# Fro116/RecommenderSystem

Measured on AMD Instinct MI355X. Metric: interactions/sec, higher is better.
Workload: dtype bf16

## Files before the change

recommendersystem_amd/csrc/elementwise.hip:

```cpp
#include "kernels.hpp"

namespace rsys {

thread_local DetScratch g_det;

__global__ void reduce_parts_kernel(const float* __restrict__ part, int nparts, long long stride, int n, float* dst) {
  const int c = blockIdx.x * blockDim.x + threadIdx.x;
  if (c >= n) return;
  float acc = 0.f;
  for (int b = 0; b < nparts; ++b) acc += part[(long long)b * stride + c];
  dst[c] += acc;
}
__global__ void reduce_parts_stage_kernel(const float* __restrict__ part, int nparts, long long stride, int n, float* out) {
  const int c = blockIdx.x * blockDim.x + threadIdx.x, chunk = blockIdx.y;
  if (c >= n) return;
  const int b0 = chunk * 32, b1 = min(nparts, b0 + 32);
  float acc = 0.f;
  for (int b = b0; b < b1; ++b) acc += part[(long long)b * stride + c];
  out[(long long)chunk * n + c] = acc;
}
int launch_reduce_parts(const float* part, int nparts, long long stride, int n, float* dst, hipStream_t s) {
  if (nparts <= 0 || n <= 0) return RSYS_OK;
  if (nparts > 64 && g_det.tmp != nullptr) {
    const int chunks = (nparts + 31) / 32;
// ... 716 lines not shown
int launch_rowdot(const T* h, const float* w, const float* b, float* out, int n, int D, hipStream_t s) {
  hipLaunchKernelGGL((rowdot_kernel<T>), dim3(div_up(n, 4)), dim3(256), 0, s, h, w, b, out, n, D);
  HIP_CHECK(hipGetLastError());
  return RSYS_OK;
}
template int launch_rowdot<bf16>(const bf16*, const float*, const float*, float*, int, int, hipStream_t);
template int launch_rowdot<float>(const float*, const float*, const float*, float*, int, int, hipStream_t);

template <typename TS>
__global__ void colsum_kernel(const TS* __restrict__ src, long long ld, long long rows, int cols, float* dst, int rows_per_block, float* part) {
  const int c = blockIdx.x * blockDim.x + threadIdx.x;
  if (c >= cols) return;
  const long long r0 = (long long)blockIdx.y * rows_per_block, r1 = min(rows, r0 + rows_per_block);
  float acc = 0.f;
  for (long long r = r0; r < r1; ++r) acc += to_f32(src[r * ld + c]);
  if (part != nullptr) part[(long long)blockIdx.y * cols + c] = acc;
  else if (acc != 0.f) atomicAdd(&dst[c], acc);
}
template <typename TS>
static int colsum_any(const TS* src, long long ld, long long rows, int cols, float* dst, hipStream_t s) {
  int rpb = (int)std::max<long long>(64, (rows + 511) / 512);
  dim3 grid(div_up(cols, 256), div_up(rows, rpb));
  float* part = det_part((long long)grid.y * cols);
  hipLaunchKernelGGL((colsum_kernel<TS>), grid, dim3(256), 0, s, src, ld, rows, cols, dst, rpb, part);
  HIP_CHECK(hipGetLastError());
  if (part != nullptr) return launch_reduce_parts(part, (int)grid.y, cols, cols, dst, s);
  return RSYS_OK;
}
int launch_colsum_add(const float* src, long long ld, long long rows, int cols, float* dst, hipStream_t s) {
  return colsum_any<float>(src, ld, rows, cols, dst, s);
}

__global__ __launch_bounds__(1024) void cast_colsum_kernel(const float* __restrict__ src, bf16* __restrict__ dst, long long rows, int D,
                                                           float* colsum, int rows_per_block, float* part) {
  __shared__ float red[2048];
  const int cg = D >> 2;
  const int c = (threadIdx.x % cg) * 4, lane_r = threadIdx.x / cg, nr = 1024 / cg;
  const long long r0 = (long long)blockIdx.x * rows_per_block, r1 = min(rows, r0 + rows_per_block);
  float4 acc = make_float4(0, 0, 0, 0);
  long long r = r0 + lane_r;
  for (; r + 3 * nr < r1; r += 4 * nr) {
    float4 v[4];
#pragma unroll
    for (int u = 0; u < 4; ++u) v[u] = *(const float4*)(src + (r + u * nr) * D + c);
#pragma unroll
    for (int u = 0; u < 4; ++u) {
      bf16x4 o; o[0] = (bf16)v[u].x; o[1] = (bf16)v[u].y; o[2] = (bf16)v[u].z; o[3] = (bf16)v[u].w;
      *(bf16x4*)(dst + (r + u * nr) * D + c) = o;
      acc.x += v[u].x; acc.y += v[u].y; acc.z += v[u].z; acc.w += v[u].w;
    }
  }
  for (; r < r1; r += nr) {
    const float4 v = *(const float4*)(src + r * D + c);
    bf16x4 o; o[0] = (bf16)v.x; o[1] = (bf16)v.y; o[2] = (bf16)v.z; o[3] = (bf16)v.w;
    *(bf16x4*)(dst + r * D + c) = o;
    acc.x += v.x; acc.y += v.y; acc.z += v.z; acc.w += v.w;
  }
  if (lane_r < 2) *(float4*)&red[lane_r * D + c] = acc;
  __syncthreads();
  for (int base = 2; base < nr; base += 2) {
    if (lane_r >= base && lane_r < base + 2) {
      float4 o = *(float4*)&red[(lane_r - base) * D + c];
      o.x += acc.x; o.y += acc.y; o.z += acc.z; o.w += acc.w;
      *(float4*)&red[(lane_r - base) * D + c] = o;
    }
    __syncthreads();
  }
  for (int cc = threadIdx.x; cc < D; cc += 1024) {
    const float v = red[cc] + (nr > 1 ? red[D + cc] : 0.f);
    if (part != nullptr) part[(long long)blockIdx.x * D + cc] = v;
    else if (v != 0.f) atomicAdd(&colsum[cc], v);
  }
}
int launch_cast_colsum(const float* src, bf16* dst, long long rows, int D, float* colsum, hipStream_t s) {
  ARG_CHECK(D % 4 == 0 && D <= 1024 && 1024 % (D >> 2) == 0, "cast_colsum: D/4 must divide 1024, D <= 1024");
  const int rpb = (int)std::max<long long>(32, (rows + 511) / 512);
  const int grid = div_up(rows, rpb);
  float* part = det_part((long long)grid * D);
  hipLaunchKernelGGL(cast_colsum_kernel, dim3(grid), dim3(1024), 0, s, src, dst, rows, D, colsum, rpb, part);
  HIP_CHECK(hipGetLastError());
  if (part != nullptr) return launch_reduce_parts(part, grid, D, D, colsum, s);
  return RSYS_OK;
}

__global__ __launch_bounds__(256) void cast_transpose_colsum_kernel(const float* __restrict__ src, bf16* __restrict__ dstT, long long rows, int D,
                                                                    long long ldt, float* colsum, int rows_per_block, float* part) {
  __shared__ unsigned short tile[64][72];
  __shared__ float red[16][64];
  const int t = threadIdx.x;
  const int lr = t >> 4, c4 = (t & 15) * 4;
  const int oc = t >> 2, or8 = (t & 3) * 16;
  const long long r0 = (long long)blockIdx.x * rows_per_block;
  const long long rend = min((rows + 63) & ~63LL, r0 + rows_per_block);
  for (int ct = 0; ct < D / 64; ++ct) {
    float4 acc = make_float4(0, 0, 0, 0);
    for (long long rb = r0; rb < rend; rb += 64) {
      float4 v[4];
#pragma unroll
      for (int i = 0; i < 4; ++i) {
        const long long r = rb + 4 * lr + i;
        v[i] = r < rows ? *(const float4*)(src + r * D + ct * 64 + c4) : make_float4(0, 0, 0, 0);
        acc.x += v[i].x; acc.y += v[i].y; acc.z += v[i].z; acc.w += v[i].w;
      }
      {
        bf16x4 o;
        o[0] = (bf16)v[0].x; o[1] = (bf16)v[1].x; o[2] = (bf16)v[2].x; o[3] = (bf16)v[3].x; *(bf16x4*)&tile[c4 + 0][4 * lr] = o;
        o[0] = (bf16)v[0].y; o[1] = (bf16)v[1].y; o[2] = (bf16)v[2].y; o[3] = (bf16)v[3].y; *(bf16x4*)&tile[c4 + 1][4 * lr] = o;
        o[0] = (bf16)v[0].z; o[1] = (bf16)v[1].z; o[2] = (bf16)v[2].z; o[3] = (bf16)v[3].z; *(bf16x4*)&tile[c4 + 2][4 * lr] = o;
        o[0] = (bf16)v[0].w; o[1] = (bf16)v[1].w; o[2] = (bf16)v[2].w; o[3] = (bf16)v[3].w; *(bf16x4*)&tile[c4 + 3][4 * lr] = o;
      }
      __syncthreads();
      {
        const uint4 q0 = *(const uint4*)&tile[oc][or8], q1 = *(const uint4*)&tile[oc][or8 + 8];
        uint4* d = (uint4*)(dstT + (long long)(ct * 64 + oc) * ldt + rb + or8);
// ... 127 lines not shown
```

recommendersystem_amd/csrc/kernels.hpp:

```cpp
#pragma once
#include "common.hpp"

namespace rsys {

struct BatchDev {
  int N, rows, S;
  const int *userid, *tmid, *gender, *source, *matchedid, *status;
  const double* time;
  const float *rating, *progress;
  const float* label[6]; const float* weight[6]; const int* position[6];
  const unsigned char *watch_mask, *rating_mask;
  const int* rope_pos;
  int *m_tmid, *m_matchedid, *m_status;
  float *m_rating, *m_progress;
  float* m_label[4]; float* m_weight[4]; int* m_position[4];
};

struct DetScratch {
  float* part = nullptr; long long cap = 0; float* tmp = nullptr; long long tmp_cap = 0;
  int part_used = 0, part_short = 0;
};
extern thread_local DetScratch g_det;
int launch_reduce_parts(const float* part, int nparts, long long stride, int n, float* dst, hipStream_t s);

// ... 26 lines not shown
                       float* f8_amax = nullptr );
template <typename T>
int launch_rmsnorm_bwd_f32(const float* g, const float* x, const float* scale, const float* rstd, const float* resid_grad,
                           float* dx_out, T* dx_out_t, float* dscale, long long rows, int D, hipStream_t s, const int* rows_dev = nullptr,
                           float* f8_amax = nullptr);

template <typename T>
int launch_dropout(const T* src, T* dst, long long n, float p, unsigned long long seed, unsigned int stream, int accumulate, hipStream_t s);

int launch_select_positions(const float* w, int N, int topk, int* idx, float* stats ,
                            int* npos_out , hipStream_t s);
int launch_select_positions_chunked(int ntask, const float* const* w, int N, int topk, int* const* idx, float* const* stats, int* const* npos_out,
                                    void* scratch, hipStream_t s);
int launch_select_positions_batch(int ntask, const float* const* w, int N, int topk, int* const* idx, float* const* stats,
                                  int* const* npos_out, hipStream_t s);

template <typename T>
int launch_gather_rows(const T* src, long long ld, const int* idx, int parity, T* dst, int n, int D, hipStream_t s);

int launch_scatter_rows_add(const float* src, const int* idx, int parity, float* dst, long long ld, int n, int D, hipStream_t s,
                            const int* npos = nullptr );

template <typename T>
int launch_ce_fwd_bwd(T* logits, long long ldl, int n, int V, const int* idx, const float* label, const float* weight,
                      const int* position, const float* stats, const int* npos, float task_w, float* loss_out, hipStream_t s);

template <typename T>
int launch_rating_tail(T* z, const T* hact, int n, int D, const float* w2, const float* b2, const int* idx,
                       const float* label, const float* weight, const float* stats, float rating_mean, float task_w,
                       int evaluate, float* loss_out , float* dw2, float* db2, float* db0, hipStream_t s,
                       const int* npos = nullptr );

int launch_colsum_add(const float* src, long long ld, long long rows, int cols, float* dst, hipStream_t s);
int launch_cast_colsum(const float* src, bf16* dst, long long rows, int D, float* colsum, hipStream_t s);
int launch_cast_transpose_colsum(const float* src, bf16* dstT, long long rows, int D, long long ldt, float* colsum, hipStream_t s);

int launch_embedding_scatter_add(const float* gx0, const BatchDev& b, int V, int D, float* gE, hipStream_t s);

int token_index_capacity(int N);
int launch_token_index_build(const int* matchedid, int N, int V, unsigned long long* keys, int* skey, int* sidx, hipStream_t s);
size_t seg_scatter_slab_floats(int N, int D);
int launch_embedding_scatter_segmented(const float* gx0, long long ldx, const int* m_matchedid, const int* skey, const int* sidx,
                                       int N, int V, int D, float* gE, float* slab, hipStream_t s);

int launch_token_union(const int* const* idx, const int* const* npos, int ntask, int NT, unsigned int* bits, int* pre, int* nsel, hipStream_t s);
int launch_selected_first(const unsigned int* bits, const int* pre, int* slot, int* sel, const int* uid, const int* tm, const int* rope_pos, int B, int T,
                          int* perm, int* uid_p, int* tm_p, int* pos_p, int* slot_p, int* sel_p, int* q_active, hipStream_t s);
template <typename T> int launch_gather_rows_sel(const T* src, long long ld, const int* sel, const int* n_dev, int cap, T* dst, int D, hipStream_t s);
template <typename T> int launch_scatter_rows_fill(const T* src, const int* slot_p, const int* q_active, int B, int Tseq, T* dst, long long ld, int D, hipStream_t s);
template <typename T> int launch_scatter_rows_sel(const T* src, const int* sel, const int* n_dev, int cap, T* dst, long long ld, int D, hipStream_t s);
template <typename T> int launch_scatter_rows_map(const T* src, const int* map, int n, T* dst, long long ld, int D, hipStream_t s);
template <typename T> int launch_gather_rows_slot(const T* compact, const int* slot, const int* idx, int parity, T* dst, int n, int D, hipStream_t s);
int launch_scatter_rows_add_slot(const float* src, const int* slot, const int* idx, int parity, const int* npos, float* compact, int n, int D, hipStream_t s);

int launch_plan_unique(const int* skey, const int* sidx, int N, int V, int* slot, int* uniq, int* tok2u, int* plan , hipStream_t s);
int launch_plan_offsets(const int* uniq, const int* plan, const int* bound_dev, int nb, int* off, hipStream_t s);
int launch_gather_rows_by_id(const float* src, long long ld, const int* ids, int sub, float* dst, int n, int D, hipStream_t s);
int launch_add_rows_by_id(const float* src, const int* ids, int sub, float* dst, long long ld, int n, int D, hipStream_t s);
int launch_add_rows_by_id_counted(const float* src, const int* ids, const int* count_dev, float* dst, long long ld, int cap, int D, hipStream_t s);
int launch_gather_items_remote(const BatchDev& b, const float* Frem, const int* tok2u, const int* plan, int D, float* x0,
                               int* uid_t, int* tm_t, hipStream_t s);
int launch_vp_meta(const int* idx, const float* label, const float* weight, const int* position, const float* stats,
                   const int* npos, float task_w, int KB, int KBmax, float* own , hipStream_t s);
int launch_add_scalar(float* dst, const float* src, hipStream_t s);
template <typename T>
int launch_vp_compact(const T* EwAll, const float* metaAll, int W, int KB, int D, T* EwC, float* metaC, int* nlive, int* pre , hipStream_t s);
// ... 104 lines not shown
```

recommendersystem_amd/csrc/model.hip:

```cpp
#include "model_internal.hpp"

namespace rsys {

static void add_tensor(Model* m, const std::string& name, int64_t rows, int64_t cols, int ndim, int64_t off, int64_t ld,
                       int map, bool trainable = true, bool frozen = false) {
  TensorInfo t{name, rows, cols, ndim, off, ld, map, trainable, frozen};
  m->by_name[name] = (int)m->tensors.size();
  m->tensors.push_back(t);
}

static void build_layout(Model* m) {
  const int D = m->D, Ip = m->Ip, I = m->I, L = m->L, hd = m->hd, H = m->H, KV = m->KV;
  const bool ft = m->cfg.finetune != 0;
  int64_t off = 0;
  auto take = [&](int64_t n) { int64_t o = off; off += pad8(n); return o; };
  m->lo.resize(L);
  if (ft) {
    for (int l = 0; l < L; ++l) { m->lo[l].la = take((int64_t)16 * D); m->lo[l].lb = take((int64_t)m->Nqkv * 16); }
  }
  const int64_t n_lora = off;
  m->o_status = take((m->cfg.vocab_status + 1) * 16);
  m->o_gender = take((m->cfg.vocab_gender + 1) * 4);
  m->o_source = take((m->cfg.vocab_source + 1) * 4);
  m->o_lin_w = take((int64_t)D * 32);
// ... 30 lines not shown
  add_tensor(m, "item_embedding.projection_layer.bias", 1, D, 1, m->o_bp, D, MAP_DIRECT, tr);
  for (int l = 0; l < L; ++l) {
    std::string p = "transformers.layers." + std::to_string(l) + ".";
    add_tensor(m, p + "attn.q_proj.weight", H * hd, D, 2, m->lo[l].wqkv, D, MAP_DIRECT, tr);
    add_tensor(m, p + "attn.k_proj.weight", KV * hd, D, 2, m->lo[l].wqkv + (int64_t)H * hd * D, D, MAP_DIRECT, tr);
    add_tensor(m, p + "attn.v_proj.weight", KV * hd, D, 2, m->lo[l].wqkv + (int64_t)(H + KV) * hd * D, D, MAP_DIRECT, tr);
    add_tensor(m, p + "attn.output_proj.weight", D, H * hd, 2, m->lo[l].wo, D, MAP_DIRECT, tr);
    if (ft) {
      add_tensor(m, p + "attn.q_proj_lora_A.weight", 8, D, 2, m->lo[l].la, D, MAP_DIRECT, true);
      add_tensor(m, p + "attn.q_proj_lora_B.weight", H * hd, 8, 2, m->lo[l].lb, 16, MAP_DIRECT, true);
      add_tensor(m, p + "attn.v_proj_lora_A.weight", 8, D, 2, m->lo[l].la + (int64_t)8 * D, D, MAP_DIRECT, true);
      add_tensor(m, p + "attn.v_proj_lora_B.weight", KV * hd, 8, 2, m->lo[l].lb + (int64_t)(H + KV) * hd * 16 + 8, 16, MAP_DIRECT, true);
    }
    add_tensor(m, p + "mlp.w1.weight", I, D, 2, m->lo[l].w13, D, MAP_W1, tr);
    add_tensor(m, p + "mlp.w2.weight", D, I, 2, m->lo[l].w2, Ip, MAP_DIRECT, tr);
    add_tensor(m, p + "mlp.w3.weight", I, D, 2, m->lo[l].w13, D, MAP_W3, tr);
    add_tensor(m, p + "sa_norm.scale", 1, D, 1, m->lo[l].sa, D, MAP_DIRECT, tr);
    add_tensor(m, p + "mlp_norm.scale", 1, D, 1, m->lo[l].mlp, D, MAP_DIRECT, tr);
  }
  add_tensor(m, "transformers.norm.scale", 1, D, 1, m->o_norm, D, MAP_DIRECT, tr);
  add_tensor(m, "rating_head.0.weight", D, D, 2, m->o_r0w, D, MAP_DIRECT, tr);
  add_tensor(m, "rating_head.0.bias", 1, D, 1, m->o_r0b, D, MAP_DIRECT, tr);
  add_tensor(m, "rating_head.2.weight", 1, D, 2, m->o_r2w, D, MAP_DIRECT, tr);
  add_tensor(m, "rating_head.2.bias", 1, 1, 1, m->o_r2b, 1, MAP_DIRECT, tr);
}

static inline int64_t internal_row(const TensorInfo& t, int64_t r) {
  if (t.map == MAP_W1) return (r / 16) * 32 + (r % 16);
  if (t.map == MAP_W3) return (r / 16) * 32 + 16 + (r % 16);
  return r;
}


int model_create(const rsys_config* cfg, int device, Model** out) {
  ARG_CHECK(cfg != nullptr && out != nullptr, "null argument");
  ARG_CHECK(cfg->embed_dim % cfg->num_heads == 0, "embed_dim % num_heads");
  ARG_CHECK(cfg->num_heads % cfg->num_kv_heads == 0, "num_heads % num_kv_heads");
  const int hd = cfg->embed_dim / cfg->num_heads;
  ARG_CHECK(hd == 16 || hd == 32 || hd == 64 || hd == 128, "head_dim must be 16/32/64/128");
  ARG_CHECK(cfg->embed_dim % 16 == 0 && cfg->embed_dim <= 2048, "embed_dim must be a multiple of 16 and <= 2048");
  ARG_CHECK(cfg->max_sequence_length % 4 == 0 && 2 * cfg->max_sequence_length <= 2048,
            "max_sequence_length must be a multiple of 4 and <= 1024");
  ARG_CHECK(cfg->max_rows >= 1, "max_rows");
  ARG_CHECK(cfg->mask_topk >= 1 && cfg->mask_topk <= cfg->max_sequence_length, "mask_topk");
  ARG_CHECK(cfg->dtype == RSYS_DTYPE_FP32 || cfg->dtype == RSYS_DTYPE_BF16 || cfg->dtype == RSYS_DTYPE_FP8, "dtype");
  ARG_CHECK(cfg->lora_dropout >= 0.f && cfg->lora_dropout < 1.f, "lora_dropout must be in [0,1)");
  ARG_CHECK(cfg->sampled_negatives == 0 || (cfg->sampled_negatives > 0 && cfg->table_shard_world >= 1),
            "sampled_negatives needs the row-sharded table (table_shard_world >= 1)");
  if (cfg->dtype == RSYS_DTYPE_FP8) {
    ARG_CHECK(!cfg->finetune, "dtype fp8: the reference converts the trunk to float8 for pretraining only (transformer.py:671)");
    ARG_CHECK(cfg->embed_dim % 128 == 0 && cfg->embed_dim >= 256 && cfg->intermediate_dim >= 129 && cfg->num_heads > 0 && cfg->num_kv_heads > 0 &&
              (cfg->num_kv_heads * (cfg->embed_dim / cfg->num_heads)) % 128 == 0 && cfg->num_heads / cfg->num_kv_heads <= 14,
              "dtype fp8 needs embed_dim % 128 == 0 (>= 256), intermediate_dim > 128, (num_kv_heads * head_dim) % 128 == 0, num_heads / num_kv_heads <= 14");
  }
  int ndev = 0;
  HIP_CHECK(hipGetDeviceCount(&ndev));
  if (ndev <= 0) { set_error("no HIP device visible: the HIP path has no CPU fallback"); return RSYS_ERR_HIP; }
  ARG_CHECK(device >= 0 && device < ndev, "device index");
  HIP_CHECK(hipSetDevice(device));
  Model* m = new Model();
  m->cfg = *cfg; m->device = device;
  m->bf16_mode = cfg->dtype == RSYS_DTYPE_BF16 || cfg->dtype == RSYS_DTYPE_FP8;
  m->fp8 = cfg->dtype == RSYS_DTYPE_FP8;
  m->esz = m->bf16_mode ? 2 : 4;
  m->L = cfg->num_layers; m->H = cfg->num_heads; m->KV = cfg->num_kv_heads; m->D = cfg->embed_dim;
  m->I = cfg->intermediate_dim; m->Ip = m->fp8 ? (m->I + 127) / 128 * 128 : (m->I + 15) / 16 * 16;
  m->S = cfg->max_sequence_length; m->T = 2 * m->S;
  m->V0 = cfg->vocab_0; m->V1 = cfg->vocab_1; m->V = m->V0 + m->V1; m->M = cfg->metadata_dim;
  m->Mp = (m->M + 63) / 64 * 64; m->K = cfg->mask_topk; m->hd = hd;
  m->Nqkv = (m->H + 2 * m->KV) * hd; m->rows_max = cfg->max_rows;
  m->sharded = cfg->table_shard_world >= 1;
  m->sh_world = m->sharded ? cfg->table_shard_world : 1; m->sh_rank = m->sharded ? cfg->table_shard_rank : 0;
  if (m->sh_world > 16 || m->sh_rank < 0 || m->sh_rank >= m->sh_world || (m->sharded && cfg->finetune)) {
    delete m;
    set_error("table_shard: rank must be in [0, world), world <= 16, and finetuning keeps the table replicated (it is frozen)");
    return RSYS_ERR_ARG;
  }
  m->row_lo = (int)((int64_t)m->sh_rank * (m->V + 1) / m->sh_world);
  m->TR = (int)((int64_t)(m->sh_rank + 1) * (m->V + 1) / m->sh_world) - m->row_lo;
  HIP_CHECK(hipStreamCreateWithFlags(&m->stream, hipStreamNonBlocking));
  HIP_CHECK(hipStreamCreateWithFlags(&m->side, hipStreamNonBlocking));
  HIP_CHECK(hipEventCreateWithFlags(&m->ev_fork, hipEventDisableTiming));
  HIP_CHECK(hipEventCreateWithFlags(&m->ev_join, hipEventDisableTiming));
  for (int k = 0; k < 4; ++k) HIP_CHECK(hipEventCreateWithFlags(&m->ev_dw[k], hipEventDisableTiming));
  HIP_CHECK(hipEventCreateWithFlags(&m->ev_sel, hipEventDisableTiming));
  build_layout(m);
  const int64_t D = m->D, N = (int64_t)m->rows_max * m->S, NT = 2 * N, KB = (int64_t)m->K * m->rows_max;
  const size_t e = m->esz;
  DALLOC(m->P, m->n_total * 4); DALLOC(m->G, m->n_total * 4);
  if (m->bf16_mode) { DALLOC(m->Sh, m->n_total * 2); DALLOC(m->ShT, m->n_total * 2); } else { m->Sh = m->P; }
  DALLOC(m->Meta, (int64_t)m->TR * m->Mp * e);
  DALLOC(m->F32, (int64_t)m->TR * D * 4); DALLOC(m->FT, (int64_t)m->TR * D * e);
  if (m->bf16_mode) {
    m->Vp = ((int64_t)m->TR + 63) / 64 * 64;
    DALLOC(m->MetaT, (int64_t)m->Mp * m->Vp * 2); DALLOC(m->dFT, (int64_t)D * m->Vp * 2);
    HIP_CHECK(hipMemset(m->MetaT, 0, (size_t)m->Mp * m->Vp * 2)); HIP_CHECK(hipMemset(m->dFT, 0, (size_t)D * m->Vp * 2));
  }
  {
    const int half = hd / 2;
    std::vector<float> c((size_t)m->T * half), s((size_t)m->T * half);
    for (int k = 0; k < half; ++k) {
      float freq = 1.0f / powf(500000.0f, (float)(2 * k) / (float)hd);
      for (int t = 0; t < m->T; ++t) { float a = (float)t * freq; c[(size_t)t * half + k] = cosf(a); s[(size_t)t * half + k] = sinf(a); }
    }
    DALLOC(m->rope_cos, c.size() * 4); DALLOC(m->rope_sin, s.size() * 4); DALLOC(m->rope_cs, c.size() * 8);
    HIP_CHECK(hipMemcpy(m->rope_cos, c.data(), c.size() * 4, hipMemcpyHostToDevice));
    HIP_CHECK(hipMemcpy(m->rope_sin, s.data(), s.size() * 4, hipMemcpyHostToDevice));
    std::vector<float> cs(c.size() * 2);
    for (size_t i = 0; i < c.size(); ++i) { cs[2 * i] = c[i]; cs[2 * i + 1] = s[i]; }
    HIP_CHECK(hipMemcpy(m->rope_cs, cs.data(), cs.size() * 4, hipMemcpyHostToDevice));
    m->rope_npos = m->T;
  }
  {
    size_t per_i = 4 * 6 + 8 + 4 * 2 + 18 * 4  + 4 * 3 + 4 * 2 + 12 * 4 ;
    DALLOC(m->batch_blob, (size_t)N * per_i + 4096);
    unsigned char* p = (unsigned char*)m->batch_blob;
    auto carve = [&](size_t bytes) { void* r = p; p += (bytes + 15) / 16 * 16; return r; };
    BatchDev& b = m->bd;
    b.time = (const double*)carve(N * 8);
    b.userid = (const int*)carve(N * 4); b.tmid = (const int*)carve(N * 4); b.gender = (const int*)carve(N * 4);
    b.source = (const int*)carve(N * 4); b.matchedid = (const int*)carve(N * 4); b.status = (const int*)carve(N * 4);
    b.rating = (const float*)carve(N * 4); b.progress = (const float*)carve(N * 4);
    for (int k = 0; k < 6; ++k) { b.label[k] = (const float*)carve(N * 4); b.weight[k] = (const float*)carve(N * 4); b.position[k] = (const int*)carve(N * 4); }
    b.m_tmid = (int*)carve(N * 4); b.m_matchedid = (int*)carve(N * 4); b.m_status = (int*)carve(N * 4);
    b.m_rating = (float*)carve(N * 4); b.m_progress = (float*)carve(N * 4);
    for (int k = 0; k < 4; ++k) { b.m_label[k] = (float*)carve(N * 4); b.m_weight[k] = (float*)carve(N * 4); b.m_position[k] = (int*)carve(N * 4); }
    b.watch_mask = nullptr; b.rating_mask = nullptr; b.rope_pos = nullptr;
    m->raw_bytes = (size_t)N * (4 * 6 + 8 + 4 * 2 + 18 * 4 + 2 + 8) + 64 * 32;
    DALLOC(m->raw_blob, m->raw_bytes);
    HIP_CHECK(hipHostMalloc((void**)&m->h_stage, m->raw_bytes, hipHostMallocDefault));
// ... 236 lines not shown
        if (a < b) RC(launch_fill_normal(m->P + t.off + (a - lo) * t.ld, (b - a) * t.ld, 0.006f, seed, stream_id, m->stream, (a - r0) * t.ld));
      }
      if (hi == (int64_t)m->V + 1) HIP_CHECK(hipMemsetAsync(m->P + t.off + (t.rows - 1) * t.ld, 0, t.cols * 4, m->stream));
      continue;
    }
    for (int64_t r0 = 0; r0 < rows; r0 += 4096) {
      int64_t nr = std::min<int64_t>(4096, rows - r0);
      RC(launch_fill_normal(m->P + t.off + r0 * t.ld, nr * t.ld, 0.006f, seed, stream_id++, m->stream));
    }
    if (t.ld != t.cols) {
      std::vector<float> host((size_t)rows * t.ld);
      HIP_CHECK(hipStreamSynchronize(m->stream));
      HIP_CHECK(hipMemcpy(host.data(), m->P + t.off, host.size() * 4, hipMemcpyDeviceToHost));
      for (int64_t r = 0; r < rows; ++r)
        for (int64_t c = t.cols; c < t.ld; ++c) host[r * t.ld + c] = 0.f;
      HIP_CHECK(hipMemcpy(m->P + t.off, host.data(), host.size() * 4, hipMemcpyHostToDevice));
    }
    if (t.map == MAP_W1 && m->Ip != m->I) {
      for (int64_t r = m->I; r < m->Ip; ++r) {
        HIP_CHECK(hipMemsetAsync(m->P + t.off + ((r / 16) * 32 + (r % 16)) * t.ld, 0, t.ld * 4, m->stream));
        HIP_CHECK(hipMemsetAsync(m->P + t.off + ((r / 16) * 32 + 16 + (r % 16)) * t.ld, 0, t.ld * 4, m->stream));
      }
    }
    if (t.name.find("embedding.weight") != std::string::npos)
      HIP_CHECK(hipMemsetAsync(m->P + t.off + (t.rows - 1) * t.ld, 0, t.cols * 4, m->stream));
  }
  RC(model_refresh_shadow(m));
  HIP_CHECK(hipStreamSynchronize(m->stream));
  return RSYS_OK;
}

static int build_meta_t(Model* m) {
  m->table_dirty = true;
  if (!m->bf16_mode) return RSYS_OK;
  TransposeBatch b; b.n = 1;
  b.job[0].src = (const bf16*)m->Meta; b.job[0].dst = (bf16*)m->MetaT; b.job[0].rows = m->TR; b.job[0].cols = m->Mp;
  b.job[0].ld_src = m->Mp; b.job[0].ld_dst = m->Vp;
  RC(launch_transpose_bf16(b, m->stream));
  HIP_CHECK(hipStreamSynchronize(m->stream));
  return RSYS_OK;
}

static int meta_write_rows(Model* m, const float* rows, int64_t nrows) {
  const int64_t Mdim = m->M;
  HIP_CHECK(hipSetDevice(m->device));
  const int64_t chunk = 4096;
  std::vector<float> hostf((size_t)chunk * m->Mp);
  std::vector<unsigned short> hosth;
  if (m->bf16_mode) hosth.resize((size_t)chunk * m->Mp);
  HIP_CHECK(hipMemset(m->Meta, 0, (size_t)m->TR * m->Mp * m->esz));
  for (int64_t r0 = 0; r0 < nrows; r0 += chunk) {
    int64_t nr = std::min(chunk, nrows - r0);
    for (int64_t r = 0; r < nr; ++r) {
      const float* src = rows + (r0 + r) * Mdim;
      if (m->bf16_mode) {
        unsigned short* d = hosth.data() + r * m->Mp;
        for (int64_t c = 0; c < Mdim; ++c) {
          uint32_t u; memcpy(&u, &src[c], 4);
          uint32_t rb = ((u >> 16) & 1u) + 0x7FFFu;
          d[c] = (unsigned short)((u + rb) >> 16);
        }
        for (int64_t c = Mdim; c < m->Mp; ++c) d[c] = 0;
      } else {
        float* d = hostf.data() + r * m->Mp;
        memcpy(d, src, Mdim * 4);
        for (int64_t c = Mdim; c < m->Mp; ++c) d[c] = 0.f;
      }
// ... 367 lines not shown
```

recommendersystem_amd/csrc/model.hpp:

```cpp
#pragma once
#include <functional>
#include <map>
#include <string>
#include <vector>

#include "../../include/rsys.h"
#include "../../include/rsys_debug.h"
#include "comm.hpp"
#include "gemm.hpp"
#include "kernels.hpp"

namespace rsys {

enum RowMap { MAP_DIRECT = 0, MAP_W1 = 1, MAP_W3 = 2 };

struct TensorInfo {
  std::string name;
  int64_t rows, cols;
  int ndim;
  int64_t off;
  int64_t ld;
  int map;
  bool trainable;
  bool frozen_table;
// ... 57 lines not shown
  std::map<std::string, int> by_name;
  int64_t o_status, o_gender, o_source, o_lin_w, o_E, o_Wp, o_r0w, o_r2w;
  int64_t o_pcos, o_psin, o_lin_b, o_bp, o_norm, o_r0b, o_r2b;
  std::vector<LayerOff> lo;
  float *P = nullptr, *G = nullptr;
  void* Sh = nullptr;
  void* ShT = nullptr;
  bool wt_dirty = true;
  bool fp8 = false;
  int64_t w8_base = 0;
  unsigned char* W8 = nullptr;
  unsigned char* W8T = nullptr;
  float* f8_wamax = nullptr;
  float* f8_aamax = nullptr;
  float* f8_desc = nullptr;
  unsigned char* a8 = nullptr;
  void* f8_jobs = nullptr; int* f8_tile_job = nullptr; int* f8_tile_first = nullptr; int f8_ntiles = 0;
  bool w8_dirty = true;
  void* sel_scratch = nullptr;
  float* rope_cs = nullptr;
  bool f8_dw = false;
  bool f8_tcopies = true;
  struct F8T { unsigned char *xn, *O, *hn, *g, *gxt, *dab, *dht, *dqkv; };
  std::vector<F8T> f8t;
  float* f8_desc_dw = nullptr;
  int64_t f8_ldt = 0;
  float* f8_dw_stage = nullptr;
  int64_t f8_dw_stage_base = 0;
  std::vector<void*> f8_keep;
  bool table_dirty = true;
  void* Meta = nullptr;
  float* F32 = nullptr;
  void* FT = nullptr;
  void* MetaT = nullptr; void* dFT = nullptr; int64_t Vp = 0;
  bool sharded = false; int sh_rank = 0, sh_world = 1;
  int row_lo = 0, TR = 0;
  rsys_comm* shard_comm = nullptr;
  int *u_slot = nullptr, *u_ids = nullptr, *u_tok = nullptr, *u_plan = nullptr , *u_bound = nullptr, *u_off = nullptr;
  int U = 0, uV = 0;
  std::vector<long long> need_off, serve_off, need_offD, serve_offD;
  int* req_ids = nullptr; long long req_cap = 0, R = 0;
  float *Frem = nullptr; float* rows_xchg = nullptr; long long xchg_cap = 0;
  void *EwAll = nullptr, *EwC = nullptr; float *metaOwn = nullptr, *metaAll = nullptr, *metaC = nullptr, *vp_max = nullptr, *vp_lmax = nullptr, *vp_sums = nullptr;
  int *vp_nlive = nullptr, *vp_pre = nullptr; float* dEwC = nullptr;
  float* metaAllT[2] = {nullptr, nullptr};
  int* h_counts = nullptr;
  hipEvent_t ev_counts = nullptr; bool counts_pending = false;
  int host_stream_syncs = 0, host_event_waits = 0;
  int64_t ldl_loc = 0; float* sumsq_E = nullptr;
  int* ss_cols = nullptr; void* ss_F = nullptr; float *ss_dF = nullptr, *ss_tl = nullptr, *ss_dt = nullptr;
  unsigned int* ss_bitmap = nullptr; int* ss_tcount = nullptr;
  unsigned long long cur_seed = 0, cur_step = 0;
  float *rope_cos = nullptr, *rope_sin = nullptr;
  int rope_npos = 0;
  std::vector<void*> allocs;
  BatchDev bd;
  void* batch_blob = nullptr;
  unsigned char* raw_blob = nullptr; unsigned char* h_stage = nullptr; size_t raw_bytes = 0;
  unsigned char* slot_blob[2] = {nullptr, nullptr}; unsigned char* slot_stage[2] = {nullptr, nullptr};
  int cur_slot = 0;
  hipStream_t copy_stream = nullptr;
  hipEvent_t ev_copy_done = nullptr;
  hipEvent_t ev_blob_free[2] = {nullptr, nullptr};
  bool blob_free_valid[2] = {false, false};
  struct PendingBatch { bool valid = false; BatchDev bd; int rows = 0; bool has_masks = false, has_rope_pos = false; int distinct_ids = 0;
                        unsigned char *d_wm = nullptr, *d_rm = nullptr; int* d_rope_pos = nullptr; } pending;
// ... 106 lines not shown
```

recommendersystem_amd/csrc/model_backward.hip:

```cpp
#include "model_internal.hpp"

namespace rsys {

static int ensure_transposes(Model* m) {
  if (!m->bf16_mode || !m->wt_dirty) return RSYS_OK;
  const int D = m->D, Ip = m->Ip;
  TransposeBatch b; b.n = 0;
  auto add = [&](int64_t off, int rows, int cols, long long ld) -> int {
    TransposeJob& j = b.job[b.n++];
    j.src = (const bf16*)m->Sh + off; j.dst = (bf16*)m->ShT + off; j.rows = rows; j.cols = cols; j.ld_src = ld; j.ld_dst = rows;
    if (b.n == 64) { int rc = launch_transpose_bf16(b, m->stream); b.n = 0; return rc; }
    return RSYS_OK;
  };
  for (int l = 0; l < m->L; ++l) {
    RC(add(m->lo[l].wqkv, m->Nqkv, D, D));
    RC(add(m->lo[l].wo, D, D, D));
    RC(add(m->lo[l].w13, 2 * Ip, D, D));
    RC(add(m->lo[l].w2, D, Ip, Ip));
  }
  RC(launch_transpose_bf16(b, m->stream));
  m->wt_dirty = false;
  return RSYS_OK;
}

// ... 336 lines not shown
        RC(launch_embedding_scatter_segmented(gx, 2LL * D, b.m_matchedid, m->u_slot, m->tok_sidx, N, m->uV, D, m->tok_T, m->scatter_slab, s));
        if (m->split_head_event) HIP_CHECK(hipStreamWaitEvent(s, m->split_head_event, 0));
        RC(launch_add_rows_by_id(m->tok_T, m->u_ids, 0, m->G + m->o_E, D, m->U, D, s));
      } else
      RC(launch_embedding_scatter_segmented(gx, 2LL * D, b.m_matchedid, m->tok_skey, m->tok_sidx, N, m->V, D, m->G + m->o_E, m->scatter_slab, s));
    }
  }
  toc(m);
  m->table_grads_pending = true;
  m->gE_clean[0] = m->gE_clean[1] = false;
  {
    GemmParams p{};
    p.A = gxt + D; p.lda = 2 * D; p.B = m->feat; p.ldb = 32; p.C = m->G + m->o_lin_w; p.ldc = 32; p.c_f32 = 1;
    p.M = D; p.N = 32; p.K = N; p.epi = EPI_ATOMIC;
    RC(gemm<T>(m, "gemm_action_dw", p, false, true, true));
  }
  RC(launch_colsum_add(gx + D, 2 * D, N, D, m->G + m->o_lin_b, s));
  {
    GemmParams p{};
    p.A = gxt + D; p.lda = 2 * D; p.B = W<T>(m, m->o_lin_w); p.ldb = 32; p.C = m->gf; p.ldc = 32; p.c_f32 = 1;
    p.M = N; p.N = 32; p.K = D; p.epi = EPI_STORE;
    RC(gemm<T>(m, "gemm_action_dx", p, false, false, true));
  }
  SmallParams sp = small_params(m);
  RC(launch_action_small_bwd(m->gf, b, sp, m->G + m->o_pcos, m->G + m->o_psin, m->G + m->o_status, m->G + m->o_gender,
                             m->G + m->o_source, s));
  toc(m);
  return RSYS_OK;
}

template <typename T>
static int finalize_grads_t(Model* m, int stage) {
  tic(m, stage == 2 ? "phase_table_bwd_gemm" : "phase_table_bwd");
  const bool direct = m->bf16_mode && m->D % 64 == 0;
  if (stage != 2 && direct) {
    RC(launch_cast_transpose_colsum(m->G + m->o_E, (bf16*)m->dFT, m->TR, m->D, m->Vp, m->G + m->o_bp, m->stream));
  } else if (stage != 2) {
    m->table_dirty = true;
    const bool fused = m->bf16_mode && m->D <= 1024 && 1024 % (m->D >> 2) == 0;
    if (fused) {
      RC(launch_cast_colsum(m->G + m->o_E, (bf16*)m->FT, m->TR, m->D, m->G + m->o_bp, m->stream));
    } else {
      if (m->bf16_mode) RC(launch_cast<bf16>(m->G + m->o_E, (bf16*)m->FT, (long long)m->TR * m->D, m->stream));
      RC(launch_colsum_add(m->G + m->o_E, m->D, m->TR, m->D, m->G + m->o_bp, m->stream));
    }
    if (m->bf16_mode) {
      TransposeBatch b; b.n = 1;
      b.job[0].src = (const bf16*)m->FT; b.job[0].dst = (bf16*)m->dFT; b.job[0].rows = m->TR; b.job[0].cols = m->D;
      b.job[0].ld_src = m->D; b.job[0].ld_dst = m->Vp;
      RC(launch_transpose_bf16(b, m->stream));
    }
  }
  if (stage != 1) {
    GemmParams p{};
    p.C = m->G + m->o_Wp; p.ldc = m->Mp; p.c_f32 = 1; p.M = m->D; p.N = m->Mp; p.epi = EPI_ATOMIC;
    if (m->bf16_mode) {
      p.A = m->dFT; p.lda = m->Vp; p.B = m->MetaT; p.ldb = m->Vp; p.K = (int)m->Vp;
      RC(gemm<T>(m, "gemm_table_dw", p, false, false, false));
    } else {
      p.A = m->G + m->o_E; p.lda = m->D; p.B = m->Meta; p.ldb = m->Mp; p.K = m->TR;
      RC(gemm<T>(m, "gemm_table_dw", p, false, true, true));
    }
  }
  toc(m);
  return RSYS_OK;
}

int model_finalize_grads(Model* m) {
  if (!m->table_grads_pending || m->cfg.finetune) return RSYS_OK;
  DetScope det(m);
  m->table_grads_pending = false;
  return m->bf16_mode ? finalize_grads_t<bf16>(m, 0) : finalize_grads_t<float>(m, 0);
}

bool model_finalize_splittable(const Model* m) { return m->table_grads_pending && !m->cfg.finetune && m->bf16_mode; }

int model_split_table_enable(Model* m, int on) {
  if (!on) { m->split_table = false; m->table_head_hook = nullptr; return RSYS_OK; }
  ARG_CHECK(!m->sharded, "split table reduce: the item table is row-sharded (its rows are reduced by their owners already)");
  ARG_CHECK(m->bf16_mode && !m->cfg.finetune, "split table reduce: bf16 training of the full model only (the fp32 mode's metadata-projection gradient reads G[E] itself)");
  HIP_CHECK(hipSetDevice(m->device));
  if (!m->tbl_R) {
    const int64_t N = (int64_t)m->rows_max * m->S;
    m->tok_cap = N + 1;
    DALLOC(m->tbl_R, (int64_t)m->TR * m->D * 4);
    DALLOC(m->tok_T, m->tok_cap * m->D * 4);
    if (!m->u_slot) { DALLOC(m->u_slot, N * 4); DALLOC(m->u_ids, (N + 1) * 4); DALLOC(m->u_tok, N * 4); DALLOC(m->u_plan, 64); }
  }
  m->split_table = true;
  return RSYS_OK;
}

int model_split_table_rows(Model* m, int64_t* rows) {
// ... 65 lines not shown
```

recommendersystem_amd/csrc/switches.hip:

```cpp
#include "switches.hpp"

#include <cstdio>
#include <cstdlib>
#include <cstring>
#include <mutex>

namespace rsys {
namespace {

struct Entry { const char* name; int Switches::*field; int dflt; };
const Entry kEntries[] = {
    {"RSYS_ATTN_DMA", &Switches::attn_dma, 1},
    {"RSYS_ATTN_KV_DMA", &Switches::attn_kv_dma, 1},
    {"RSYS_ATTN_KV32", &Switches::attn_kv32, 1},
    {"RSYS_ATTN_FWD32", &Switches::attn_fwd32, 0},
    {"RSYS_GEMM_KERNEL", &Switches::gemm_kernel, -1},
    {"RSYS_GEMM_KERNEL_TN", &Switches::gemm_kernel_tn, -1},
    {"RSYS_GEMM_KERNEL_NT_SPLITK", &Switches::gemm_kernel_nt_splitk, -1},
    {"RSYS_GEMM_KERNEL_MIX", &Switches::gemm_kernel_mix, 1},
    {"RSYS_GEMM8C_HALF", &Switches::gemm8c_half, 1},
    {"RSYS_GEMM4P", &Switches::gemm4p, 1},
    {"RSYS_GEMM4K", &Switches::gemm4k, 1},
    {"RSYS_GEMM8C", &Switches::gemm8c, 1},
    {"RSYS_GEMM_REVERSE", &Switches::gemm_reverse, 1},
    {"RSYS_GEMM_PATCH", &Switches::gemm_patch, 1},
    {"RSYS_TABLE_TAIL", &Switches::table_tail, 1},
    {"RSYS_DW_GROUP", &Switches::dw_group, 1},
    {"RSYS_DET_DW_GROUP", &Switches::det_dw_group, 1},
    {"RSYS_SPARSE_TOP", &Switches::sparse_top, 1},
    {"RSYS_TOP_ORDER", &Switches::top_order, 1},
    {"RSYS_SELECT_ASIDE", &Switches::select_aside, 0},
    {"RSYS_SELECT_CHUNKED", &Switches::select_chunked, 1},
    {"RSYS_SIDE_STREAM", &Switches::side_stream, 0},
    {"RSYS_SCATTER_ATOMIC", &Switches::scatter_atomic, 0},
    {"RSYS_F8_DW", &Switches::f8_dw, 1},
    {"RSYS_F8_DW_ROUND_BF16", &Switches::f8_dw_round_bf16, 0},
    {"RSYS_F8_DEBUG_KEEP", &Switches::f8_debug_keep, 0},
    {"RSYS_FORCE_RCCL", &Switches::force_rccl, 0},
    {"RSYS_DEBUG_8P", &Switches::debug_8p, 0},
    {"RSYS_DEBUG_8G_SPLITK", &Switches::debug_8g_splitk, 0},
    {"RSYS_DEBUG_8T_SPLITK", &Switches::debug_8t_splitk, 0},
    {"RSYS_DEBUG_EPI", &Switches::debug_epi, -1},
    {"RSYS_DEBUG_F8_CAST_WAVES", &Switches::debug_f8_cast_waves, 4},
    {"RSYS_DEBUG_NORM_BWD_GRID", &Switches::debug_norm_bwd_grid, 1024},
    {"RSYS_DEBUG_NORM_BWD_WAVES", &Switches::debug_norm_bwd_waves, 0},
    {"RSYS_DEBUG_ADAMW", &Switches::debug_adamw, 0},
};

Switches g_sw;
bool g_parsed = false;
std::mutex g_mu;

void parse_locked() {
  for (const Entry& e : kEntries) {
    const char* v = getenv(e.name);
    g_sw.*(e.field) = (v && *v) ? atoi(v) : e.dflt;
  }
  g_parsed = true;
}
// ... 26 lines not shown
```

recommendersystem_amd/csrc/switches.hpp:

```cpp
#pragma once

namespace rsys {

struct Switches {
  int attn_dma;
  int attn_kv_dma;
  int attn_fwd32;
  int attn_kv32;
  int gemm_kernel;
  int gemm_kernel_tn;
  int gemm_kernel_nt_splitk;
  int gemm_kernel_mix;
  int gemm8c_half;
  int gemm4p;
  int gemm4k;
  int gemm8c;
  int gemm_reverse;
  int gemm_patch;
  int table_tail;
  int dw_group;
  int det_dw_group;
  int sparse_top;
  int top_order;
  int select_aside;
  int select_chunked;
  int side_stream;
  int scatter_atomic;
  int f8_dw;
  int f8_dw_round_bf16;
  int f8_debug_keep;
  int force_rccl;
  int debug_8p;
  int debug_8g_splitk;
  int debug_8t_splitk;
  int debug_epi;
  int debug_f8_cast_waves;
  int debug_norm_bwd_grid;
  int debug_adamw;
  int debug_norm_bwd_waves;
};

const Switches& sw();
void switches_parse();
int switches_describe(char* buf, int cap);

}
```

Before: 1.610 million.

## Compute table weight gradient from row-major bf16 gradient instead of transposed copies

By default in non-deterministic bf16 mode, the table weight-gradient GEMM now reads the row-major bf16 cast gradient (FT) against Meta using transposed-operand flags, rather than first transposing the gradient into dFT and using the pre-transposed MetaT. This removes the cast-transpose or transpose pass over the table gradient. The fused cast+colsum kernel gains a leading-dimension argument so it can run on column chunks when D is a multiple of 1024. The old transposed path stays behind a switch and is still used in deterministic mode. The risk is that the GEMM with transposed operands may run slower than the NN form it replaces.

Result: no change. 1.619 million, median of 6 (+0.6%).

```diff
diff --git a/recommendersystem_amd/csrc/elementwise.hip b/recommendersystem_amd/csrc/elementwise.hip
--- a/recommendersystem_amd/csrc/elementwise.hip
+++ b/recommendersystem_amd/csrc/elementwise.hip
@@ -772,7 +772,7 @@
 }
 
 __global__ __launch_bounds__(1024) void cast_colsum_kernel(const float* __restrict__ src, bf16* __restrict__ dst, long long rows, int D,
-                                                           float* colsum, int rows_per_block, float* part) {
+                                                           long long ld, float* colsum, int rows_per_block, float* part) {
   __shared__ float red[2048];
   const int cg = D >> 2;
   const int c = (threadIdx.x % cg) * 4, lane_r = threadIdx.x / cg, nr = 1024 / cg;
@@ -782,18 +782,18 @@
   for (; r + 3 * nr < r1; r += 4 * nr) {
     float4 v[4];
 #pragma unroll
-    for (int u = 0; u < 4; ++u) v[u] = *(const float4*)(src + (r + u * nr) * D + c);
+    for (int u = 0; u < 4; ++u) v[u] = *(const float4*)(src + (r + u * nr) * ld + c);
 #pragma unroll
     for (int u = 0; u < 4; ++u) {
       bf16x4 o; o[0] = (bf16)v[u].x; o[1] = (bf16)v[u].y; o[2] = (bf16)v[u].z; o[3] = (bf16)v[u].w;
-      *(bf16x4*)(dst + (r + u * nr) * D + c) = o;
+      *(bf16x4*)(dst + (r + u * nr) * ld + c) = o;
       acc.x += v[u].x; acc.y += v[u].y; acc.z += v[u].z; acc.w += v[u].w;
     }
   }
   for (; r < r1; r += nr) {
-    const float4 v = *(const float4*)(src + r * D + c);
+    const float4 v = *(const float4*)(src + r * ld + c);
     bf16x4 o; o[0] = (bf16)v.x; o[1] = (bf16)v.y; o[2] = (bf16)v.z; o[3] = (bf16)v.w;
-    *(bf16x4*)(dst + r * D + c) = o;
+    *(bf16x4*)(dst + r * ld + c) = o;
     acc.x += v.x; acc.y += v.y; acc.z += v.z; acc.w += v.w;
   }
   if (lane_r < 2) *(float4*)&red[lane_r * D + c] = acc;
@@ -812,14 +812,20 @@
     else if (v != 0.f) atomicAdd(&colsum[cc], v);
   }
 }
+bool cast_colsum_eligible(int D) { return D % 4 == 0 && (D <= 1024 ? 1024 % (D >> 2) == 0 : D % 1024 == 0); }
 int launch_cast_colsum(const float* src, bf16* dst, long long rows, int D, float* colsum, hipStream_t s) {
-  ARG_CHECK(D % 4 == 0 && D <= 1024 && 1024 % (D >> 2) == 0, "cast_colsum: D/4 must divide 1024, D <= 1024");
+  ARG_CHECK(cast_colsum_eligible(D), "cast_colsum: D/4 must divide 1024 (D <= 1024) or D a multiple of 1024");
   const int rpb = (int)std::max<long long>(32, (rows + 511) / 512);
-  const int grid = div_up(rows, rpb);
-  float* part = det_part((long long)grid * D);
-  hipLaunchKernelGGL(cast_colsum_kernel, dim3(grid), dim3(1024), 0, s, src, dst, rows, D, colsum, rpb, part);
-  HIP_CHECK(hipGetLastError());
-  if (part != nullptr) return launch_reduce_parts(part, grid, D, D, colsum, s);
+  const int grid = div_up(rows, rpb), Dw = std::min(D, 1024);
+  for (int c0 = 0; c0 < D; c0 += Dw) {
+    float* part = det_part((long long)grid * Dw);
+    hipLaunchKernelGGL(cast_colsum_kernel, dim3(grid), dim3(1024), 0, s, src + c0, dst + c0, rows, Dw, (long long)D, colsum + c0, rpb, part);
+    HIP_CHECK(hipGetLastError());
+    if (part != nullptr) {
+      const int rc = launch_reduce_parts(part, grid, Dw, Dw, colsum + c0, s);
+      if (rc != RSYS_OK) return rc;
+    }
+  }
   return RSYS_OK;
 }
 
diff --git a/recommendersystem_amd/csrc/kernels.hpp b/recommendersystem_amd/csrc/kernels.hpp
--- a/recommendersystem_amd/csrc/kernels.hpp
+++ b/recommendersystem_amd/csrc/kernels.hpp
@@ -82,6 +82,7 @@
                        const int* npos = nullptr );
 
 int launch_colsum_add(const float* src, long long ld, long long rows, int cols, float* dst, hipStream_t s);
+bool cast_colsum_eligible(int D);
 int launch_cast_colsum(const float* src, bf16* dst, long long rows, int D, float* colsum, hipStream_t s);
 int launch_cast_transpose_colsum(const float* src, bf16* dstT, long long rows, int D, long long ldt, float* colsum, hipStream_t s);
 
diff --git a/recommendersystem_amd/csrc/model.hip b/recommendersystem_amd/csrc/model.hip
--- a/recommendersystem_amd/csrc/model.hip
+++ b/recommendersystem_amd/csrc/model.hip
@@ -86,6 +86,11 @@
 }
 
 
+static int alloc_meta_t(Model* m) {
+  DALLOC(m->MetaT, (int64_t)m->Mp * m->Vp * 2); DALLOC(m->dFT, (int64_t)m->D * m->Vp * 2);
+  return RSYS_OK;
+}
+
 int model_create(const rsys_config* cfg, int device, Model** out) {
   ARG_CHECK(cfg != nullptr && out != nullptr, "null argument");
   ARG_CHECK(cfg->embed_dim % cfg->num_heads == 0, "embed_dim % num_heads");
@@ -145,11 +150,9 @@
   if (m->bf16_mode) { DALLOC(m->Sh, m->n_total * 2); DALLOC(m->ShT, m->n_total * 2); } else { m->Sh = m->P; }
   DALLOC(m->Meta, (int64_t)m->TR * m->Mp * e);
   DALLOC(m->F32, (int64_t)m->TR * D * 4); DALLOC(m->FT, (int64_t)m->TR * D * e);
-  if (m->bf16_mode) {
-    m->Vp = ((int64_t)m->TR + 63) / 64 * 64;
-    DALLOC(m->MetaT, (int64_t)m->Mp * m->Vp * 2); DALLOC(m->dFT, (int64_t)D * m->Vp * 2);
-    HIP_CHECK(hipMemset(m->MetaT, 0, (size_t)m->Mp * m->Vp * 2)); HIP_CHECK(hipMemset(m->dFT, 0, (size_t)D * m->Vp * 2));
-  }
+  m->dw_transposed = m->bf16_mode && sw().table_dw_transposed != 0;
+  m->Vp = ((int64_t)m->TR + 63) / 64 * 64;
+  if (m->bf16_mode) RC(alloc_meta_t(m));
   {
     const int half = hd / 2;
     std::vector<float> c((size_t)m->T * half), s((size_t)m->T * half);
@@ -452,7 +455,7 @@
 
 static int build_meta_t(Model* m) {
   m->table_dirty = true;
-  if (!m->bf16_mode) return RSYS_OK;
+  if (m->MetaT == nullptr) return RSYS_OK;
   TransposeBatch b; b.n = 1;
   b.job[0].src = (const bf16*)m->Meta; b.job[0].dst = (bf16*)m->MetaT; b.job[0].rows = m->TR; b.job[0].cols = m->Mp;
   b.job[0].ld_src = m->Mp; b.job[0].ld_dst = m->Vp;
diff --git a/recommendersystem_amd/csrc/model.hpp b/recommendersystem_amd/csrc/model.hpp
--- a/recommendersystem_amd/csrc/model.hpp
+++ b/recommendersystem_amd/csrc/model.hpp
@@ -113,6 +113,7 @@
   void* Meta = nullptr;
   float* F32 = nullptr;
   void* FT = nullptr;
+  bool dw_transposed = false;
   void* MetaT = nullptr; void* dFT = nullptr; int64_t Vp = 0;
   bool sharded = false; int sh_rank = 0, sh_world = 1;
   int row_lo = 0, TR = 0;
diff --git a/recommendersystem_amd/csrc/model_backward.hip b/recommendersystem_amd/csrc/model_backward.hip
--- a/recommendersystem_amd/csrc/model_backward.hip
+++ b/recommendersystem_amd/csrc/model_backward.hip
@@ -392,19 +392,20 @@
 template <typename T>
 static int finalize_grads_t(Model* m, int stage) {
   tic(m, stage == 2 ? "phase_table_bwd_gemm" : "phase_table_bwd");
-  const bool direct = m->bf16_mode && m->D % 64 == 0;
+  const bool transposed = m->bf16_mode && (m->dw_transposed || m->deterministic);
+  const bool direct = transposed && m->D % 64 == 0;
   if (stage != 2 && direct) {
     RC(launch_cast_transpose_colsum(m->G + m->o_E, (bf16*)m->dFT, m->TR, m->D, m->Vp, m->G + m->o_bp, m->stream));
   } else if (stage != 2) {
     m->table_dirty = true;
-    const bool fused = m->bf16_mode && m->D <= 1024 && 1024 % (m->D >> 2) == 0;
+    const bool fused = m->bf16_mode && cast_colsum_eligible(m->D);
     if (fused) {
       RC(launch_cast_colsum(m->G + m->o_E, (bf16*)m->FT, m->TR, m->D, m->G + m->o_bp, m->stream));
     } else {
       if (m->bf16_mode) RC(launch_cast<bf16>(m->G + m->o_E, (bf16*)m->FT, (long long)m->TR * m->D, m->stream));
       RC(launch_colsum_add(m->G + m->o_E, m->D, m->TR, m->D, m->G + m->o_bp, m->stream));
     }
-    if (m->bf16_mode) {
+    if (transposed) {
       TransposeBatch b; b.n = 1;
       b.job[0].src = (const bf16*)m->FT; b.job[0].dst = (bf16*)m->dFT; b.job[0].rows = m->TR; b.job[0].cols = m->D;
       b.job[0].ld_src = m->D; b.job[0].ld_dst = m->Vp;
@@ -414,11 +415,11 @@
   if (stage != 1) {
     GemmParams p{};
     p.C = m->G + m->o_Wp; p.ldc = m->Mp; p.c_f32 = 1; p.M = m->D; p.N = m->Mp; p.epi = EPI_ATOMIC;
-    if (m->bf16_mode) {
+    if (transposed) {
       p.A = m->dFT; p.lda = m->Vp; p.B = m->MetaT; p.ldb = m->Vp; p.K = (int)m->Vp;
       RC(gemm<T>(m, "gemm_table_dw", p, false, false, false));
     } else {
-      p.A = m->G + m->o_E; p.lda = m->D; p.B = m->Meta; p.ldb = m->Mp; p.K = m->TR;
+      p.A = m->bf16_mode ? (const void*)m->FT : (const void*)(m->G + m->o_E); p.lda = m->D; p.B = m->Meta; p.ldb = m->Mp; p.K = m->TR;
       RC(gemm<T>(m, "gemm_table_dw", p, false, true, true));
     }
   }
diff --git a/recommendersystem_amd/csrc/switches.hip b/recommendersystem_amd/csrc/switches.hip
--- a/recommendersystem_amd/csrc/switches.hip
+++ b/recommendersystem_amd/csrc/switches.hip
@@ -25,6 +25,7 @@
     {"RSYS_GEMM_REVERSE", &Switches::gemm_reverse, 1},
     {"RSYS_GEMM_PATCH", &Switches::gemm_patch, 1},
     {"RSYS_TABLE_TAIL", &Switches::table_tail, 1},
+    {"RSYS_TABLE_DW_TRANSPOSED", &Switches::table_dw_transposed, 0},
     {"RSYS_DW_GROUP", &Switches::dw_group, 1},
     {"RSYS_DET_DW_GROUP", &Switches::det_dw_group, 1},
     {"RSYS_SPARSE_TOP", &Switches::sparse_top, 1},
diff --git a/recommendersystem_amd/csrc/switches.hpp b/recommendersystem_amd/csrc/switches.hpp
--- a/recommendersystem_amd/csrc/switches.hpp
+++ b/recommendersystem_amd/csrc/switches.hpp
@@ -18,6 +18,7 @@
   int gemm_reverse;
   int gemm_patch;
   int table_tail;
+  int table_dw_transposed;
   int dw_group;
   int det_dw_group;
   int sparse_top;
```
